# ChenJiahao031008/EAO-Fusion

Hardware: AMD Instinct MI355X
Metric: ORB kpts/s (640x480, 1k feat) + local-BA residuals/s (20 KF x 3k pts) (higher is better)
Workload: dtype u8; 1 GPU; ORBextractor FAST+rBRIEF, 640x480, 8-level pyramid, nFeatures 1000, batch=64 synthetic frames per GPU (BASELINE configs[1]); parallelism=frames sharded per GPU, no data-path collective

## Files before the change

eao_fusion_amd/csrc/orb.hip:

```cpp
#include "orb_internal.h"

using namespace eao::orb;

namespace {

__constant__ __align__(16) signed char c_pattern[1024] = {
#include "orb_pattern.inc"
};

constexpr int kResizeRows = 4;
__device__ __forceinline__ unsigned udot2w(unsigned a, unsigned b) {
    typedef unsigned short us2 __attribute__((ext_vector_type(2)));
    return __builtin_amdgcn_udot2(__builtin_bit_cast(us2, a), __builtin_bit_cast(us2, b), 0u, false);
}

struct ResizeLevel { int w, h, pitch, off; };
struct ResizeArgs {
    ResizeLevel D, S;
    double invX, invY;
    int srcIsInput;
    int pyrFrameBytes;
    int G;
    float invG;
    int frameAffinity;
// ... 535 lines not shown
    if (MODE == 1) {
        const unsigned a = e.left ? L[0] : L[1], b = e.left ? L[1] : L[2];
        W0 = __builtin_amdgcn_perm(L[1], L[0], e.selA);
        W1 = __builtin_amdgcn_perm(b, a, e.selB);
        W2 = __builtin_amdgcn_perm(b, a, e.selC);
    }
    constexpr unsigned T0 = 18u | 34u << 8 | 49u << 16 | 55u << 24, T1 = 49u | 34u << 8 | 18u << 16;
    hres[0] = __builtin_amdgcn_udot4(__builtin_amdgcn_alignbyte(W1, W0, 1), T0, __builtin_amdgcn_udot4(__builtin_amdgcn_alignbyte(W2, W1, 1), T1, 0, false), false);
    hres[1] = __builtin_amdgcn_udot4(__builtin_amdgcn_alignbyte(W1, W0, 2), T0, __builtin_amdgcn_udot4(__builtin_amdgcn_alignbyte(W2, W1, 2), T1, 0, false), false);
    hres[2] = __builtin_amdgcn_udot4(__builtin_amdgcn_alignbyte(W1, W0, 3), T0, __builtin_amdgcn_udot4(__builtin_amdgcn_alignbyte(W2, W1, 3), T1, 0, false), false);
    hres[3] = __builtin_amdgcn_udot4(W1, T0, __builtin_amdgcn_udot4(W2, T1, 0, false), false);
}

template <int MODE>
__device__ __forceinline__ void blur_strip(const uint8_t* __restrict__ src, int pitch, uint8_t* __restrict__ dst, int dpitch, int x4, int y0, int w, int h) {
    BlurEdge e = {};
    if (MODE == 1) e = blur_edge(x4, w);
    constexpr int NP = (kBlurRows + 6) / 2;
    constexpr int PF = MODE == 2 ? 1 : 3;
    unsigned raw[NP][2][3];
    auto fetch = [&](int m) {
#pragma unroll
        for (int q = 0; q < 2; q++) {
            int t = y0 - 3 + 2 * m + q;
            t = t < 0 ? -t : t;
            t = min(t, 2 * h - 2 - t);
            blur_load<MODE>(src, __umul24(t, pitch), x4, w, e, raw[m][q]);
        }
    };
#pragma unroll
    for (int m = 0; m < PF; m++) fetch(m);
    unsigned P[4][4];
#pragma unroll
    for (int m = 0; m < NP; m++) {
        if (m + PF < NP) fetch(m + PF);
        unsigned hr[2][4];
        blur_hpass<MODE>(raw[m][0], e, hr[0]);
        blur_hpass<MODE>(raw[m][1], e, hr[1]);
#pragma unroll
        for (int i = 0; i < 4; i++) P[m & 3][i] = hr[0][i] | (hr[1][i] << 16);
        if (m >= 3) {
#pragma unroll
            for (int q = 0; q < 2; q++) {
                const unsigned K0 = q ? 18u << 16 : (18u | 34u << 16), K1 = q ? (34u | 49u << 16) : (49u | 55u << 16),
                               K2 = q ? (55u | 49u << 16) : (49u | 34u << 16), K3 = q ? (34u | 18u << 16) : 18u;
                unsigned sv[4];
#pragma unroll
                for (int i = 0; i < 4; i++)
                    sv[i] = udot2(P[(m - 3) & 3][i], K0, udot2(P[(m - 2) & 3][i], K1, udot2(P[(m - 1) & 3][i], K2, udot2(P[m & 3][i], K3, 32768u))));
                const u16x2 lim = {255, 255};
                const u16x2 pa = __builtin_elementwise_min(__builtin_bit_cast(u16x2, __builtin_amdgcn_perm(sv[1], sv[0], 0x07060302u)), lim);
                const u16x2 pb = __builtin_elementwise_min(__builtin_bit_cast(u16x2, __builtin_amdgcn_perm(sv[3], sv[2], 0x07060302u)), lim);
                const unsigned packed = __builtin_amdgcn_perm(__builtin_bit_cast(unsigned, pb), __builtin_bit_cast(unsigned, pa), 0x06040200u);
                const int y = y0 + 2 * (m - 3) + q;
                *reinterpret_cast<unsigned*>(dst + (unsigned)(__umul24(y, dpitch) + x4)) = packed;
            }
        }
    }
}

__global__ __launch_bounds__(256) void k_blur7(const Geom* __restrict__ g, ImgSrc s, uint8_t* __restrict__ blur, int f0, int src0Aligned, int frameAffinity) {
    const int lane = threadIdx.x & 31;
    int f = blockIdx.y, bxi = blockIdx.x;
    if (frameAffinity) {
        const unsigned b = blockIdx.x + gridDim.x * blockIdx.y, xcd = b & 7, slot = b >> 3;
        f = (int)(xcd + 8 * (slot / gridDim.x)); bxi = (int)(slot % gridDim.x);
    }
    f += f0;
    int l = 0;
    while (l + 1 < g->nlevels && bxi >= g->L[l + 1].tileBase) l++;
    const LevelGeom L = g->L[l];
    const int strip = (bxi - L.tileBase) * kBlurStripsPerWg + (int)(threadIdx.x >> 5);
    const int x4 = (strip % L.tilesX) * kBlurSegW + lane * 4;
    const int y0 = (strip / L.tilesX) * kBlurRows;
    if (x4 >= L.w || y0 >= L.h) return;
    int pitch;
    const uint8_t* src = level_ptr(g, s, l, f, &pitch);
    uint8_t* dst = blur + (long long)f * g->pyrFrameBytes + L.off;
    if (l == 0 && !src0Aligned) blur_strip<2>(src, pitch, dst, L.pitch, x4, y0, L.w, L.h);
    else if (__any(x4 < 4 || x4 + 7 > L.w)) blur_strip<1>(src, pitch, dst, L.pitch, x4, y0, L.w, L.h);
    else blur_strip<0>(src, pitch, dst, L.pitch, x4, y0, L.w, L.h);
}

__device__ __forceinline__ int half_sum_i32(int v, int half) {
    v += __builtin_amdgcn_update_dpp(0, v, 0xB1, 0xF, 0xF, true);
    v += __builtin_amdgcn_update_dpp(0, v, 0x4E, 0xF, 0xF, true);
    v += __builtin_amdgcn_update_dpp(0, v, 0x141, 0xF, 0xF, true);
    v += __builtin_amdgcn_update_dpp(0, v, 0x140, 0xF, 0xF, true);
    v += __builtin_amdgcn_update_dpp(0, v, 0x142, 0xA, 0xF, true);
    const int lo = __builtin_amdgcn_readlane(v, 31), hi = __builtin_amdgcn_readlane(v, 63);
    return half ? hi : lo;
}

constexpr int kUmaxTab[16] = {15, 15, 15, 15, 14, 14, 14, 13, 13, 12, 11, 10, 9, 8, 6, 3};

__device__ __forceinline__ void sincos_f32_via_f64(float angle, float* sn, float* cs) {
    const double x = (double)angle;
    const int k = (int)(x * 0.63661977236758134308 + 0.5);
    const double kd = (double)k;
    const double r = (x - kd * 1.57079632673412561417e+00) - kd * 6.07710050650619224932e-11;
    const double z = r * r;
    const double ps = -1.66666666666666324348e-01 + z * (8.33333333332248946124e-03 + z * (-1.98412698298579493134e-04 +
                      z * (2.75573137070700676789e-06 + z * (-2.50507602534068634195e-08 + z * 1.58969099521155010221e-10))));
    const double sr = r + r * z * ps;
    const double pc = 4.16666666666666019037e-02 + z * (-1.38888888888741095749e-03 + z * (2.48015872894767294178e-05 +
                      z * (-2.75573143513906633035e-07 + z * (2.08757232129817482790e-09 + z * -1.13596475577881948265e-11))));
    const double cr = 1.0 - 0.5 * z + z * z * pc;
    double sv = (k & 1) ? cr : sr, cv = (k & 1) ? sr : cr;
    if (k & 2) sv = -sv;
    if ((k + 1) & 2) cv = -cv;
    *sn = (float)sv;
    *cs = (float)cv;
}

__device__ __forceinline__ float fast_atan2_deg(float y, float x) {
    const float p1 = 0.9997878412794807f * (float)(180 / 3.1415926535897932384626433832795);
    const float p3 = -0.3258083974640975f * (float)(180 / 3.1415926535897932384626433832795);
    const float p5 = 0.1555786518463281f * (float)(180 / 3.1415926535897932384626433832795);
    const float p7 = -0.04432655554792128f * (float)(180 / 3.1415926535897932384626433832795);
    const float eps = (float)2.2204460492503131e-16;
    const float ax = fabsf(x), ay = fabsf(y);
    const bool ge = ax >= ay;
    const float c = (ge ? ay : ax) / ((ge ? ax : ay) + eps);
    const float c2 = c * c;
    const float poly = (((p7 * c2 + p5) * c2 + p3) * c2 + p1) * c;
    float a = ge ? poly : 90.f - poly;
    if (x < 0) a = 180.f - a;
    if (y < 0) a = 360.f - a;
    return a;
}

constexpr int kDescKp = 8;
constexpr int kPR = 18, kPW = 10, kPRows = 2 * kPR + 1, kPLoads = (kPRows + 2) / 3;
constexpr int kMR = 15, kMW = 9, kMRows = 2 * kMR + 1, kMLoads = (kMRows + 2) / 3;

__global__ __launch_bounds__(256) void k_orient_describe(const Geom* __restrict__ g, ImgSrc s, const uint8_t* __restrict__ blur,
                                                         const unsigned* __restrict__ levelkps, const int* __restrict__ levelcnt,
                                                         eao_keypoint* __restrict__ kps, uint8_t* __restrict__ desc,
                                                         int* __restrict__ nout, int cap, int f0, int nlevels, int lFirst, int lEnd, int writeN,
                                                         int frameAffinity) {
    const int lane = threadIdx.x & 63, wv = __builtin_amdgcn_readfirstlane(threadIdx.x >> 6);
    const int hl = lane & 31, half = lane >> 5;
    const int bx = frameAffinity ? (int)(blockIdx.x >> 3) : (int)blockIdx.x;
    const int fy = frameAffinity ? (int)((blockIdx.x & 7) + 8 * blockIdx.y) : (int)blockIdx.y;
    int p = bx * 4 + wv;
    const int f = fy + f0;
    int total, l, kbase, pbase, cntl;
    {
        int cinc = lane < lEnd ? levelcnt[f * nlevels + lane] : 0;
        int pinc = (cinc + 1) >> 1;
        cinc += __builtin_amdgcn_update_dpp(0, cinc, 0x111, 0xF, 0xF, true);
        pinc += __builtin_amdgcn_update_dpp(0, pinc, 0x111, 0xF, 0xF, true);
        cinc += __builtin_amdgcn_update_dpp(0, cinc, 0x112, 0xF, 0xF, true);
        pinc += __builtin_amdgcn_update_dpp(0, pinc, 0x112, 0xF, 0xF, true);
        cinc += __builtin_amdgcn_update_dpp(0, cinc, 0x114, 0xF, 0xF, true);
        pinc += __builtin_amdgcn_update_dpp(0, pinc, 0x114, 0xF, 0xF, true);
        cinc += __builtin_amdgcn_update_dpp(0, cinc, 0x118, 0xF, 0xF, true);
        pinc += __builtin_amdgcn_update_dpp(0, pinc, 0x118, 0xF, 0xF, true);
        total = __builtin_amdgcn_readlane(cinc, 15);
        if (lFirst > 0) p += __builtin_amdgcn_readlane(pinc, lFirst - 1);
        l = (int)__popcll(__ballot(lane < nlevels && pinc <= p));
        const int lprev = min(l, kMaxLevels) - 1;
        pbase = l > 0 ? __builtin_amdgcn_readlane(pinc, lprev) : 0;
        kbase = l > 0 ? __builtin_amdgcn_readlane(cinc, lprev) : 0;
        cntl = __builtin_amdgcn_readlane(cinc, min(l, kMaxLevels - 1)) - kbase;
    }
// ... 148 lines not shown
    const int row = (int)vL;
    const float minZ = A.mb, minD = -3, maxD = A.mbf / minZ;
    const float minU = uL - maxD, maxU = uL - minD;
    float outU = -1.0f, outD = -1.0f;
    int outS = -1;
    if (!(maxU < 0)) {
        const uint4 a0 = A.dl[2 * iL], a1 = A.dl[2 * iL + 1];
        unsigned best = 0xFFFFFFFFu;
        for (int iR = lane; iR < A.nr; iR += 64) {
            const eao_keypoint kr = A.kr[iR];
            const float r = 2.0f * A.scale[kr.octave];
            const int maxr = (int)ceilf(kr.y + r), minr = (int)floorf(kr.y - r);
            if (row < minr || row > maxr) continue;
            if (kr.octave < levelL - 1 || kr.octave > levelL + 1) continue;
            if (!(kr.x >= minU && kr.x <= maxU)) continue;
            const uint4 b0 = A.dr[2 * iR], b1 = A.dr[2 * iR + 1];
            const unsigned d = __popc(a0.x ^ b0.x) + __popc(a0.y ^ b0.y) + __popc(a0.z ^ b0.z) + __popc(a0.w ^ b0.w) +
                               __popc(a1.x ^ b1.x) + __popc(a1.y ^ b1.y) + __popc(a1.z ^ b1.z) + __popc(a1.w ^ b1.w);
            best = min(best, (d << 16) | (unsigned)iR);
        }
        for (int dlt = 32; dlt >= 1; dlt >>= 1) best = min(best, (unsigned)__shfl_xor((int)best, dlt));
        const int bestDist = (int)(best >> 16);
        if (best != 0xFFFFFFFFu && bestDist < refc::TH_HIGH) {
            const int bestIdxR = (int)(best & 0xFFFF);
            const float uR0 = A.kr[bestIdxR].x;
            const float sf = A.invScale[levelL];
            const int suL = (int)roundf(uL * sf), svL = (int)roundf(vL * sf), suR0 = (int)roundf(uR0 * sf);
            const int w = 5, Lw = 5;
            int pl, pr;
            const uint8_t* imgL = level_ptr(g, sl, levelL, A.frame, &pl);
            const uint8_t* imgR = level_ptr(g, sr, levelL, A.frame, &pr);
            const int lw = g->L[levelL].w, lh = g->L[levelL].h;
            const float iniu = (float)(suR0 + Lw - w), endu = (float)(suR0 + Lw + w + 1);
            if (!(iniu < 0 || endu >= (float)lw)) {
                const int cL = px_reflect(imgL, pl, lw, lh, suL, svL);
                int dL0 = 0, dL1 = 0, px0x = 0, px0y = 0, px1x = 0, px1y = 0;
                const bool has1 = lane + 64 < 121;
                px0y = lane / 11; px0x = lane - px0y * 11;
                dL0 = px_reflect(imgL, pl, lw, lh, suL - w + px0x, svL - w + px0y) - cL;
                if (has1) {
                    px1y = (lane + 64) / 11; px1x = lane + 64 - px1y * 11;
                    dL1 = px_reflect(imgL, pl, lw, lh, suL - w + px1x, svL - w + px1y) - cL;
                }
                int dists[11];
                int bestSad = 0x7FFFFFFF, bestinc = 0;
#pragma unroll
                for (int inc = -5; inc <= 5; inc++) {
                    const int cR = px_reflect(imgR, pr, lw, lh, suR0 + inc, svL);
                    int sacc = abs(dL0 - (px_reflect(imgR, pr, lw, lh, suR0 + inc - w + px0x, svL - w + px0y) - cR));
                    if (has1) sacc += abs(dL1 - (px_reflect(imgR, pr, lw, lh, suR0 + inc - w + px1x, svL - w + px1y) - cR));
                    for (int dlt = 32; dlt >= 1; dlt >>= 1) sacc += __shfl_xor(sacc, dlt);
                    dists[inc + 5] = sacc;
                    if (sacc < bestSad) { bestSad = sacc; bestinc = inc; }
                }
                if (!(bestinc == -Lw || bestinc == Lw)) {
                    float dist1 = 0, dist2 = 0, dist3 = 0;
#pragma unroll
                    for (int k = 0; k < 11; k++) {
                        if (k == Lw + bestinc - 1) dist1 = (float)dists[k];
                        if (k == Lw + bestinc) dist2 = (float)dists[k];
                        if (k == Lw + bestinc + 1) dist3 = (float)dists[k];
                    }
                    const float deltaR = (dist1 - dist3) / (2.0f * (dist1 + dist3 - 2.0f * dist2));
                    if (!(deltaR < -1 || deltaR > 1)) {
                        float bestuR = A.scale[levelL] * ((float)suR0 + (float)bestinc + deltaR);
                        float disparity = uL - bestuR;
                        if (disparity >= 0 && disparity < maxD) {
                            if (disparity <= 0) { disparity = 0.01f; bestuR = uL - 0.01f; }
                            outD = A.mbf / disparity;
                            outU = bestuR;
                            outS = bestSad;
                        }
                    }
                }
            }
        }
    }
    if (lane == 0) { A.uRight[iL] = outU; A.depth[iL] = outD; A.sad[iL] = outS; }
}

namespace eao {
namespace orb {

eao_status enqueue(eao_orb* h, const uint8_t* d_img, int pitch0, long long fs0, int batch, eao_keypoint* d_kps,
                   uint8_t* d_desc, int cap, int* d_n, hipStream_t st) {
    const Geom& g = h->geom;
    eao::Range rAll("eao_orb_extract: enqueue");
    ImgSrc s;
    s.img0 = d_img; s.pitch0 = pitch0; s.fs0 = fs0; s.pyr = h->d_pyr.p;
    h->lastSrc = s; h->lastBatch = batch; h->lastComplete = false; h->pyrFrame = -1;
    const bool prof = h->profiling;
    hipEvent_t* ev = nullptr;
    if (prof) {
        if (h->evUsed + kProfEvents > h->evs.size()) {
            const size_t old = h->evs.size();
            h->evs.resize(old + kProfEvents * 16, nullptr);
            for (size_t i = old; i < h->evs.size(); i++) EAO_HIP(hipEventCreate(&h->evs[i]));
        }
        ev = &h->evs[h->evUsed];
        h->evUsed += kProfEvents;
        EAO_HIP(hipEventRecord(ev[0], st));
    }
    eao_status so;
    if (h->evLastValid && h->lastStream != st) {
        if ((so = order_behind_last_call(h, st))) return so;
    }
    h->lastStream = st;
    EAO_HIP(hipEventRecord(h->evStart, st));
    const hipStream_t ss = h->side;
    const int cells0 = g.L[0].nCells;
    const bool early0 = !prof && g.nlevels > 1 && g.L[0].cellBase == 0 && cells0 < g.totalCells;
    const int aff = (batch & 7) == 0 ? 1 : 0;
    auto fast = [&](hipStream_t str, int first, int end) {
        eao::Range rg("orb: FAST cells");
        const bool whole = first == 0 && end == g.totalCells, narrow = g.fastStride == 48;
        auto* kern = whole ? (narrow ? k_fast_cells<true, 48> : k_fast_cells<true, kTileStrideWide>)
                           : (narrow ? k_fast_cells<false, 48> : k_fast_cells<false, kTileStrideWide>);
        hipLaunchKernelGGL(kern, dim3(128 * ((end - first + 127) / 128), batch), dim3(64), g.fastLdsBytes, str, h->d_geom.p, h->d_cells.p, s,
                           h->d_cellcand.p, h->d_cellcnt.p, 0, first, end, aff);
    };
    const int mid = early0 && batch >= 48 && g.nlevels > 3 ? 3 : 0;
    const bool qtEarly = mid > 0 && batch <= 96;
    const int src0Aligned = ((((uintptr_t)s.img0 | (uintptr_t)s.pitch0 | (uintptr_t)(batch > 1 ? s.fs0 : 0)) & 3) == 0) ? 1 : 0;
    auto quadtree = [&](hipStream_t str, int lFirst, int nLev) {
        eao::Range rg("orb: quad-tree");
        launch_quadtree(h, str, batch, 0, lFirst, nLev);
    };
    auto blur = [&]() -> eao_status {
        EAO_HIP(hipStreamWaitEvent(ss, h->evFork, 0));
        if (prof) EAO_HIP(hipEventRecord(ev[6], ss));
        { eao::Range rg("orb: blur"); hipLaunchKernelGGL(k_blur7, dim3(g.totalTiles, batch), dim3(256), 0, ss, h->d_geom.p, s, h->d_blur.p, 0, src0Aligned, aff); }
        if (prof) EAO_HIP(hipEventRecord(ev[7], ss));
        EAO_HIP(hipEventRecord(h->evJoin, ss));
        return EAO_OK;
    };
    auto describe = [&](hipStream_t str, int lFirst, int lEnd, int writeN) {
        eao::Range rg("orb: orientation + description");
        int pairs = 0;
        for (int l = lFirst; l < lEnd; l++) pairs += eao::cdiv(g.L[l].listCap, 2);
        const int gx = std::max(1, eao::cdiv(std::min(pairs, eao::cdiv(cap, 2) + g.nlevels), 4));
        hipLaunchKernelGGL(k_orient_describe, aff ? dim3(8 * gx, batch / 8) : dim3(gx, batch), dim3(256), 0, str,
                           h->d_geom.p, s, h->d_blur.p, h->d_levelkps.p, h->d_levelcnt.p, d_kps, d_desc, d_n, cap, 0, g.nlevels, lFirst, lEnd, writeN, aff);
    };
    if (h->pyrFused && batch <= 32) {
        auto pyramid = [&] {
            eao::Range rg("orb: pyramid");
            hipLaunchKernelGGL(k_pyramid_fused, dim3(h->pyr.tilesX * h->pyr.tilesY, 1, batch), dim3(kPyrThreads), h->pyrLds, st, h->pyr, s, 0);
        };
        if (prof) {
            pyramid();
            EAO_HIP(hipEventRecord(ev[1], st));
            EAO_HIP(hipEventRecord(h->evFork, st));
            if ((so = blur())) return so;
            EAO_HIP(hipStreamWaitEvent(st, h->evJoin, 0));
            EAO_HIP(hipEventRecord(ev[9], st));
            fast(st, 0, g.totalCells);
            EAO_HIP(hipEventRecord(ev[2], st));
            quadtree(st, 0, g.nlevels);
            EAO_HIP(hipEventRecord(ev[3], st));
            EAO_HIP(hipEventRecord(ev[4], st));
        } else {
            EAO_HIP(hipStreamWaitEvent(ss, h->evStart, 0));
            fast(ss, 0, cells0);
            quadtree(ss, 0, 1);
            pyramid();
            EAO_HIP(hipEventRecord(h->evFork, st));
            if ((so = blur())) return so;
            fast(st, cells0, g.totalCells);
            quadtree(st, 1, g.nlevels - 1);
            EAO_HIP(hipStreamWaitEvent(st, h->evJoin, 0));
        }
    } else {
        if (early0) {
            EAO_HIP(hipStreamWaitEvent(ss, h->evStart, 0));
            fast(ss, 0, cells0);
        }
        for (int l = 1; l < g.nlevels; l++) {
            const int G4 = eao::cdiv(g.L[l].w, 4);
            ResizeArgs ra;
            ra.G = G4; ra.invG = 1.0f / (float)G4;
            ra.D = {g.L[l].w, g.L[l].h, g.L[l].pitch, g.L[l].off};
            ra.S = {g.L[l - 1].w, g.L[l - 1].h, g.L[l - 1].pitch, g.L[l - 1].off};
            ra.invX = 1. / ((double)g.L[l].w / g.L[l - 1].w); ra.invY = 1. / ((double)g.L[l].h / g.L[l - 1].h);
            ra.srcIsInput = l == 1; ra.pyrFrameBytes = g.pyrFrameBytes;
            ra.frameAffinity = aff;
            { eao::Range rg("orb: pyramid"); hipLaunchKernelGGL(k_resize, dim3(eao::cdiv(G4 * eao::cdiv(g.L[l].h, kResizeRows), 64), 1, batch), dim3(64), 0, st, ra, s, 0); }
            if (l == mid - 1) {
                EAO_HIP(hipEventRecord(h->evMid, st));
                EAO_HIP(hipStreamWaitEvent(ss, h->evMid, 0));
                fast(ss, cells0, g.L[mid].cellBase);
                if (qtEarly) quadtree(ss, 0, mid);
            }
        }
        if (early0 && !qtEarly) EAO_HIP(hipEventRecord(h->evFast0, ss));
        if (prof) {
            EAO_HIP(hipEventRecord(ev[1], st));
            EAO_HIP(hipEventRecord(h->evFork, st));
            if ((so = blur())) return so;
            EAO_HIP(hipStreamWaitEvent(st, h->evJoin, 0));
            EAO_HIP(hipEventRecord(ev[9], st));
            fast(st, 0, g.totalCells);
            EAO_HIP(hipEventRecord(ev[2], st));
        } else {
            EAO_HIP(hipEventRecord(h->evFork, st));
            fast(st, early0 ? (mid ? g.L[mid].cellBase : cells0) : 0, g.totalCells);
            if ((so = blur())) return so;
            if (early0 && !qtEarly) EAO_HIP(hipStreamWaitEvent(st, h->evFast0, 0));
        }
        quadtree(st, qtEarly ? mid : 0, g.nlevels - (qtEarly ? mid : 0));
        if (prof) EAO_HIP(hipEventRecord(ev[3], st));
        EAO_HIP(hipStreamWaitEvent(st, h->evJoin, 0));
        if (prof) EAO_HIP(hipEventRecord(ev[4], st));
    }
    describe(st, 0, g.nlevels, 1);
// ... 200 lines not shown
```

eao_fusion_amd/csrc/orb_host.hip:

```cpp
#include "orb_internal.h"

using namespace eao::orb;

namespace eao {
namespace orb {

eao_status build_geometry(eao_orb* h, int W, int H) {
    const eao_orb_cfg& c = h->cfg;
    Geom& g = h->geom;
    std::memset(&g, 0, sizeof(g));
    g.nlevels = c.nlevels; g.W = W; g.H = H;
    g.iniTh = c.ini_th_fast; g.minTh = c.min_th_fast;
    for (int i = 0; i < 16; i++) g.umax[i] = h->umax[i];
    h->cells.clear();
    int off = 0, kpBase = 0, candBase = 0, tileBase = 0, maxCell = 0, scanCap = 0, maxList = 0, maxSw = 0, maxSh = 0;
    for (int l = 0; l < c.nlevels; l++) {
        LevelGeom& L = g.L[l];
        const float s = h->invScale[l];
        L.w = cv_round((float)W * s);
        L.h = cv_round((float)H * s);
        EAO_REQUIRE(L.w < 4096 && L.h < 4096, "level %d is %dx%d: coordinates are packed in 12 bits", l, L.w, L.h);
        const int maxBX = L.w - kEdge + 3, maxBY = L.h - kEdge + 3;
        const float width = (float)(maxBX - kMinBorder), height = (float)(maxBY - kMinBorder);
        const int nCols = (int)(width / (float)refc::FAST_CELL), nRows = (int)(height / (float)refc::FAST_CELL);
// ... 84 lines not shown
                    capv[c.nlevels - 1] = std::max(capv[c.nlevels - 1], r1 - r0);
                    for (int l = 1; l < c.nlevels; l++) { table[(size_t)l * nT + col].x = o0[l]; table[(size_t)l * nT + col].y = o1[l]; }
                    table[(size_t)(c.nlevels - 1) * nT + col].z = r0; table[(size_t)(c.nlevels - 1) * nT + col].w = r1;
                    for (int l = c.nlevels - 1; l >= 1; l--) {
                        int q0 = l > 1 ? o0[l - 1] : 0x7FFFFFFF, q1 = l > 1 ? o1[l - 1] : 0;
                        if (r1 > r0) {
                            const double inv = isX ? P.L[l].invX : P.L[l].invY;
                            const int sn = isX ? g.L[l - 1].w : g.L[l - 1].h;
                            q0 = std::min(q0, pyr_src_ofs(r0, inv, sn));
                            q1 = std::max(q1, std::min(pyr_src_ofs(r1 - 1, inv, sn) + 1, sn - 1) + 1);
                        }
                        if (q0 > q1) q0 = q1 = 0;
                        capv[l - 1] = std::max(capv[l - 1], q1 - q0);
                        table[(size_t)(l - 1) * nT + col].z = q0; table[(size_t)(l - 1) * nT + col].w = q1;
                        r0 = q0; r1 = q1;
                    }
                }
            };
            axis(P.tilesX, kPyrTW, true, capW);
            axis(P.tilesY, kPyrTH, false, capH);
            size_t lds = 0;
            int coefCap = 1;
            for (int l = 0; l < c.nlevels; l++) {
                P.L[l].ldsW = ((capW[l] + 3) & ~3) + 16; P.L[l].ldsH = capH[l] + 1;
                P.L[l].ldsOff = (int)lds;
                lds += ((size_t)P.L[l].ldsW * P.L[l].ldsH + 15) & ~(size_t)15;
                coefCap = std::max(coefCap, std::max(capW[l], capH[l]));
            }
            coefCap = (coefCap + 7) & ~3;
            P.coefOff = (int)lds; P.coefCap = coefCap;
            lds += (size_t)coefCap * 16;
            h->pyrLds = lds;
            h->pyrFused = lds <= 64 * 1024 && h->cfg.scale_factor <= 2.0f;
            for (int l = 1; l < c.nlevels; l++)
                if (P.L[l].invX > 2.0 || P.L[l].invY > 2.0) h->pyrFused = false;
            if (h->pyrFused) {
                std::vector<int2> cxv, cyv;
                for (int l = 1; l < c.nlevels; l++) {
                    P.L[l].coefXOff = (int)cxv.size(); P.L[l].coefYOff = (int)cyv.size();
                    for (int d = 0; d < g.L[l].w; d++) { int o; unsigned w2; resize_coef_host(d, P.L[l].invX, g.L[l - 1].w, true, &o, &w2); cxv.push_back(make_int2(o, (int)w2)); }
                    for (int d = 0; d < g.L[l].h; d++) { int o; unsigned w2; resize_coef_host(d, P.L[l].invY, g.L[l - 1].h, false, &o, &w2); cyv.push_back(make_int2(o, (int)w2)); }
                }
                eao_status st2 = h->d_pyrRanges.reserve(table.size());
                if (st2) return st2;
                if ((st2 = h->d_pyrCoef.reserve(cxv.size() + cyv.size()))) return st2;
                EAO_HIP(hipMemcpy(h->d_pyrRanges.p, table.data(), table.size() * sizeof(int4), hipMemcpyHostToDevice));
                EAO_HIP(hipMemcpy(h->d_pyrCoef.p, cxv.data(), cxv.size() * sizeof(int2), hipMemcpyHostToDevice));
                EAO_HIP(hipMemcpy(h->d_pyrCoef.p + cxv.size(), cyv.data(), cyv.size() * sizeof(int2), hipMemcpyHostToDevice));
                P.ranges = h->d_pyrRanges.p;
                P.coefX = h->d_pyrCoef.p; P.coefY = h->d_pyrCoef.p + cxv.size();
            }
        }
    }
    g.scanCap = scanCap;
    g.fastMaxTested = std::max(1, (maxSw - 6) * (maxSh - 6));
    g.fastStride = maxSw + 3 <= 48 ? 48 : kTileStrideWide;
    g.fastTileBytes = ((maxSh * g.fastStride) + 15) & ~15;
    g.fastLdsBytes = g.fastTileBytes + ((2 * g.fastMaxTested + 15) & ~15) + ((((maxSw - 4) * (maxSh - 4)) + 15) & ~15) + 64;
    h->quadLds = (size_t)maxList * (2 * sizeof(short4) + sizeof(int) * kQtNodeInts) + (size_t)scanCap * sizeof(int);
    g.qtNodesGlobal = 0; g.qtNodeFrameBytes = 0;
    if (h->quadLds > 100 * 1024) {
        g.qtNodesGlobal = 1;
        long long noff = 0;
        for (int l = 0; l < c.nlevels; l++) {
            g.L[l].nodeOff = noff;
            noff += (long long)align256((size_t)g.L[l].listCap * (2 * sizeof(short4) + sizeof(int) * kQtNodeInts) + (size_t)scanCap * sizeof(int));
        }
        g.qtNodeFrameBytes = noff;
        h->quadLds = 0;
    }
    h->quadLds = (h->quadLds + 15) & ~(size_t)15;
    g.qtKeysOff = (int)h->quadLds;
    const size_t kQtLdsCand = std::min<size_t>(8192, std::max<size_t>(2048, ((size_t)h->cfg.nfeatures * 4 + 63) & ~(size_t)63));
    g.qtLdsCand = (int)std::min<size_t>(kQtLdsCand, h->quadLds < 76 * 1024 ? (76 * 1024 - h->quadLds) / 6 : 0) & ~7;
    h->quadLds += (size_t)g.qtLdsCand * 6;
    if (g.qtNodesGlobal) { g.qtLdsCand = 0; h->quadLds = 0; }
    {
        float cf[7]; double sum = 0;
        for (int i = 0; i < 7; i++) { double x = i - 3; cf[i] = (float)std::exp(-0.5 / 4.0 * x * x); sum += cf[i]; }
        const int expect[7] = {18, 34, 49, 55, 49, 34, 18};
        for (int i = 0; i < 7; i++)
            if (cv_round((double)(float)(cf[i] * (1. / sum)) * 256.0) != expect[i]) { eao::set_error("gaussian taps mismatch"); return EAO_ERR_INTERNAL; }
    }
    { eao_status st = h->d_geom.reserve(1); if (st) return st; }
    EAO_HIP(hipMemcpyAsync(h->d_geom.p, &g, sizeof(Geom), hipMemcpyHostToDevice, h->stream));
    { eao_status st = h->d_cells.reserve(h->cells.size()); if (st) return st; }
    EAO_HIP(hipMemcpyAsync(h->d_cells.p, h->cells.data(), h->cells.size() * sizeof(CellDesc), hipMemcpyHostToDevice, h->stream));
    EAO_HIP(eao::wait_latency(h->stream));
    { eao_status sq = quadtree_reserve_lds(h->quadLds); if (sq) return sq; }
    h->geomValid = true;
    h->batchCap = 0;
    return EAO_OK;
}

eao_status ensure(eao_orb* h, int W, int H, int batch, hipStream_t caller) {
    eao_status st = eao::require_device();
    if (st) return st;
    if (!h->stream && batch > 0) {
        int least = 0, greatest = 0, p = 0;
        const bool follow = (uintptr_t)caller != kNoCallerStream && !(getenv("EAO_STREAM_PRIORITY") && !atoi(getenv("EAO_STREAM_PRIORITY"))) &&
                            hipDeviceGetStreamPriorityRange(&least, &greatest) == hipSuccess && least != greatest && hipStreamGetPriority(caller, &p) == hipSuccess;
        (void)hipGetLastError();
        auto make = [&](hipStream_t* q) -> hipError_t {
            if ((uintptr_t)caller == kNoCallerStream) return eao::create_stream(q, eao::StreamClass::Latency);
            if (!follow || p == 0) return hipStreamCreateWithFlags(q, hipStreamNonBlocking);
            return hipStreamCreateWithPriority(q, hipStreamNonBlocking, p);
        };
        EAO_HIP(make(&h->stream));
        EAO_HIP(hipEventCreateWithFlags(&h->evStart, hipEventDisableTiming));
        EAO_HIP(hipEventCreateWithFlags(&h->evLast, hipEventDisableTiming));
        EAO_HIP(make(&h->spacer));
        EAO_HIP(make(&h->side));
        for (hipEvent_t* e : {&h->evFork, &h->evFast0, &h->evMid, &h->evJoin}) EAO_HIP(hipEventCreateWithFlags(e, hipEventDisableTiming));
    }
    if (!h->d_dbg && getenv("EAO_DEBUG_STAMPS")) {
        EAO_HIP(hipMalloc(&h->d_dbg, 16 * kMaxLevels * sizeof(long long)));
        EAO_HIP(hipMemset(h->d_dbg, 0, 16 * kMaxLevels * sizeof(long long)));
    }
    if (!h->geomValid || h->geom.W != W || h->geom.H != H) {
        st = build_geometry(h, W, H);
        if (st) return st;
    }
    if (batch > h->batchCap) {
        const Geom& g = h->geom;
        const size_t B = batch;
#define RES(buf, cnt) do { st = h->buf.reserve(cnt); if (st) return st; } while (0)
        RES(d_pyr, B * g.pyrFrameBytes);
        RES(d_blur, B * g.pyrFrameBytes);
        RES(d_cellcand, B * (size_t)g.totalCells * g.cellCap);
        RES(d_cellcnt, B * g.totalCells);
        RES(d_cand, B * (size_t)g.totalCandCap);
        RES(d_nodeof, B * (size_t)g.totalCandCap);
        if (g.qtNodesGlobal) RES(d_qtnodes, B * (size_t)g.qtNodeFrameBytes);
        RES(d_levelkps, B * (size_t)g.totalKpCap);
        RES(d_levelcnt, B * g.nlevels);
        RES(d_candcnt, B * g.nlevels);
#undef RES
        h->batchCap = batch;
    }
    return EAO_OK;
}

eao_status order_behind_last_call(eao_orb* h, hipStream_t st) {
    if (h->evLastRecorded) EAO_HIP(hipStreamWaitEvent(st, h->evLast, 0));
    else EAO_HIP(hipDeviceSynchronize());
    h->everyCallEvent = true;
    return EAO_OK;
}

void stream_release(eao_orb* h) {
    for (eao_orb::StreamSlot& sl : h->slots) {
        if (sl.evOut && sl.submitted) (void)hipEventSynchronize(sl.evOut);
        if (sl.pinIn) (void)hipHostFree(sl.pinIn);
        if (sl.pinOut) (void)hipHostFree(sl.pinOut);
        if (sl.dIn) (void)hipFree(sl.dIn);
        if (sl.dOut) (void)hipFree(sl.dOut);
        if (sl.evIn) (void)hipEventDestroy(sl.evIn);
        if (sl.evOut) (void)hipEventDestroy(sl.evOut);
        if (sl.evDone) (void)hipEventDestroy(sl.evDone);
    }
    h->slots.clear();
    for (hipStream_t* q : {&h->sUp, &h->sRun, &h->sDown})
        if (*q) { (void)hipStreamSynchronize(*q); (void)hipStreamDestroy(*q); *q = nullptr; }
}

eao_status wait_last_extraction(eao_orb* h) {
// ... 365 lines not shown
```

eao_fusion_amd/csrc/orb_internal.h:

```cpp
#pragma once

#include <algorithm>
#include <atomic>
#include <cmath>
#include <cstdlib>
#include <cstring>
#include <vector>

#include "common.h"


namespace eao {
namespace orb {

constexpr int kMaxLevels = 16;
constexpr int kEdge = refc::EDGE_THRESHOLD;
constexpr int kMinBorder = kEdge - 3;
constexpr int kTile = 72;
constexpr int kTileStrideWide = 80;
constexpr int kMaxIni = 16;
constexpr size_t kPinnedOutMax = 1 << 20;
constexpr int kFastXcdRun = 0;

struct LevelGeom {
    int w, h, pitch, off;
    int cellBase, nCells;
    int quota;
    int nIni, boxH;
    float hX;
    int listCap;
    int kpBase;
    int candBase, candCap;
    int tileBase, tilesX;
    long long nodeOff;
    int scaledPatch;
    float scale;
};

struct Geom {
    int nlevels, W, H;
    int totalCells, cellCap;
    int totalKpCap, totalCandCap, totalTiles;
    int pyrFrameBytes;
    int iniTh, minTh;
    int scanCap;
    int qtLdsCand, qtKeysOff;
    int qtNodesGlobal;
    long long qtNodeFrameBytes;
    int fastMaxTested, fastTileBytes, fastLdsBytes, fastStride;
    int umax[16];
    LevelGeom L[kMaxLevels];
};

struct CellDesc {
    short level, x0, y0, sw, sh, offX, offY, pad;
};

struct ImgSrc {
    const uint8_t* img0;
    int pitch0;
    long long fs0;
    uint8_t* pyr;
};

__device__ __forceinline__ const uint8_t* level_ptr(const Geom* g, const ImgSrc& s, int l, int f, int* pitch) {
    if (l == 0) {
        *pitch = s.pitch0;
        return s.img0 + (long long)f * s.fs0;
    }
    *pitch = g->L[l].pitch;
    return s.pyr + (long long)f * g->pyrFrameBytes + g->L[l].off;
}

constexpr int kPyrTW = 128, kPyrTH = 32;
constexpr int kPyrThreads = 256;
struct PyrLevel { int w, h, pitch, off; double invX, invY; int ldsOff, ldsW, ldsH; int coefXOff, coefYOff; };
struct PyrArgs {
    int nlevels, tilesX, tilesY, pyrFrameBytes;
    int coefOff;
    int coefCap;
    PyrLevel L[kMaxLevels];
    const int4* ranges;
    const int2* coefX;
    const int2* coefY;
};

constexpr int kQTSmall = 1024, kQTLarge = 256;
constexpr int kQtNodeInts = 2 + 2 + 2 + 4 + 4 + 5;

constexpr size_t kProfEvents = 10;


inline void resize_coef_host(int d, double inv, int slimit, bool clampHi, int* ofs, unsigned* wpair) {
    float fr = (float)(((double)d + 0.5) * inv - 0.5);
    int o = (int)std::floor(fr);
    fr -= (float)o;
    if (clampHi) {
        if (o < 0) { fr = 0; o = 0; }
        if (o >= slimit - 1) { fr = 0; o = slimit - 1; }
    }
    const int w0 = std::min(std::max((int)std::lrintf((1.f - fr) * 2048.f), -32768), 32767);
    const int w1 = std::min(std::max((int)std::lrintf(fr * 2048.f), -32768), 32767);
    *ofs = o;
    *wpair = ((unsigned)w0 & 0xFFFFu) | ((unsigned)w1 << 16);
}

__host__ __device__ inline int pyr_src_ofs(int d, double inv, int sn) {
    float fr = (float)(((double)d + 0.5) * inv - 0.5);
    int o = (int)floorf(fr);
    return o < 0 ? 0 : (o > sn - 1 ? sn - 1 : o);
}
__host__ __device__ inline int pyr_first_at_least(int bound, double inv, int sn, int dn) {
    if (bound <= 0) return 0;
    int d = (int)((double)bound / inv);
    d = d < 0 ? 0 : (d > dn ? dn : d);
    while (d > 0 && pyr_src_ofs(d - 1, inv, sn) >= bound) d--;
    while (d < dn && pyr_src_ofs(d, inv, sn) < bound) d++;
    return d;
}

constexpr int kBlurRows = 16;
constexpr int kBlurSegW = 128;
constexpr int kBlurStripsPerWg = 8;
inline int cv_round(double v) { return (int)std::lrint(v); }

}
}

struct eao_orb {
    using Geom = eao::orb::Geom; using CellDesc = eao::orb::CellDesc; using PyrArgs = eao::orb::PyrArgs; using ImgSrc = eao::orb::ImgSrc;
    eao_orb_cfg cfg;
    std::vector<float> scale, invScale, sigma2, invSigma2;
    std::vector<int> quota;
    int umax[16];
    Geom geom;
    bool geomValid = false;
    int batchCap = 0;
    std::vector<CellDesc> cells;
    size_t quadLds = 0;
    eao::DevBuf<int4> d_pyrRanges;
    eao::DevBuf<int2> d_pyrCoef;
    PyrArgs pyr;
    size_t pyrLds = 0;
    bool pyrFused = false;
    hipStream_t stream = nullptr;
    hipStream_t side = nullptr;
    hipStream_t spacer = nullptr;
    bool evLastValid = false;
    hipStream_t lastStream = nullptr;
    hipEvent_t evLast = nullptr;
    bool everyCallEvent = false, evLastRecorded = false;
    hipEvent_t evStart = nullptr, evFork = nullptr, evJoin = nullptr, evFast0 = nullptr, evMid = nullptr;
    eao::DevBuf<Geom> d_geom;
    eao::DevBuf<CellDesc> d_cells;
    eao::DevBuf<uint8_t> d_pyr, d_blur, d_in;
    eao::DevBuf<unsigned> d_cellcand, d_cand, d_levelkps;
    eao::DevBuf<unsigned short> d_nodeof;
    eao::DevBuf<unsigned char> d_qtnodes;
    eao::DevBuf<int> d_cellcnt, d_levelcnt, d_candcnt, d_nout;
    eao::DevBuf<eao_keypoint> d_kps;
    unsigned char* pinOut = nullptr;
    size_t pinOutCap = 0;
    unsigned char* pinUp = nullptr;
    size_t pinUpCap = 0;
    eao::DevBuf<uint8_t> d_desc;
    eao::DevBuf<float> d_xyr;
    eao::DevBuf<unsigned char> d_stereo;
    unsigned char* pinPyr = nullptr;
    size_t pinPyrCap = 0;
    eao_orb_level_view pyrViews[eao::orb::kMaxLevels] = {};
    int pyrFrame = -1, pyrBorder = -1;
    int autoPyrBorder = -1;
    bool lastComplete = false;
    ImgSrc lastSrc{};
    int lastBatch = 0;
    bool profiling = false;
    long long* d_dbg = nullptr;
    std::vector<hipEvent_t> evs;
    size_t evUsed = 0;
    struct StreamSlot {
        unsigned char* pinIn = nullptr; unsigned char* pinOut = nullptr;
        unsigned char* pinOutDev = nullptr;
        unsigned char* dIn = nullptr; unsigned char* dOut = nullptr;
        hipEvent_t evIn = nullptr, evDone = nullptr, evOut = nullptr;
        int batch = 0;
        bool submitted = false;
    };
    std::vector<StreamSlot> slots;
    hipStream_t sUp = nullptr, sRun = nullptr, sDown = nullptr;
    int sW = 0, sH = 0, sB = 0, sCap = 0, sPitch = 0;
    size_t sInBytes = 0, sOutBytes = 0, sOffK = 0, sOffD = 0;
};

namespace eao {
namespace orb {
constexpr uintptr_t kNoCallerStream = ~(uintptr_t)0;
eao_status ensure(eao_orb* h, int W, int H, int batch, hipStream_t caller = (hipStream_t)kNoCallerStream);
eao_status order_behind_last_call(eao_orb* h, hipStream_t st);
void stream_release(eao_orb* h);
eao_status wait_last_extraction(eao_orb* h);
eao_status upload_frames(eao_orb* h, const uint8_t* img, int width, int height, int stride, long long frame_stride, int batch);
eao_status enqueue(eao_orb* h, const uint8_t* d_img, int pitch0, long long fs0, int batch, eao_keypoint* d_kps, uint8_t* d_desc, int cap, int* d_n, hipStream_t st);
eao_status enqueue_pyramid_export(eao_orb* h, int frame, int border);
void launch_quadtree(const eao_orb* h, hipStream_t str, int nb, int f0, int lFirst, int nLev);
eao_status quadtree_reserve_lds(size_t bytes);
}
}
```

Before: 271.1 million kpts/s.

## Compute 7-tap Gaussian blur as int8 MFMA matrix products with precomputed tap tables

Adds a blur kernel that expresses the separable 7-tap Gaussian as two int8 MFMA matrix multiplies (horizontal then vertical) over 32x32 tiles. It uses host-built, deduplicated tap matrices that fold reflect-101 borders into the weights, and splits intermediates into hi/lo byte planes to keep exact integer results. The aim is to move blur arithmetic off the vector ALUs onto matrix cores. In exchange it adds LDS staging, table loads, and a VALU fallback for levels too small for the tiling. It is enabled by default and can be disabled with an environment variable.

```diff
diff --git a/eao_fusion_amd/csrc/orb.hip b/eao_fusion_amd/csrc/orb.hip
--- a/eao_fusion_amd/csrc/orb.hip
+++ b/eao_fusion_amd/csrc/orb.hip
@@ -641,6 +641,141 @@
     else blur_strip<0>(src, pitch, dst, L.pitch, x4, y0, L.w, L.h);
 }
 
+typedef int bm_v4i __attribute__((ext_vector_type(4)));
+typedef int bm_v16i __attribute__((ext_vector_type(16)));
+typedef bm_v4i bm_v4i_a4 __attribute__((aligned(4)));
+struct BlurMPacked { bm_v4i hi, lo; };
+
+constexpr int kBlurMLdsPitch = 80;
+__device__ __forceinline__ void blur_m_load(const uint8_t* __restrict__ src, int pitch, int h, int blk, unsigned ws, int lane, bm_v4i raw[2]) {
+#pragma unroll
+    for (int k = 0; k < 2; k++) {
+        const int y = min(max(kBlurMTile * blk + 16 * k + (lane >> 2), 0), h - 1);
+        raw[k] = *reinterpret_cast<const bm_v4i_a4*>(src + (unsigned)(__umul24(y, pitch) + ws + 16 * (lane & 3)));
+    }
+}
+
+__device__ __forceinline__ BlurMPacked blur_m_stage1(const bm_v4i raw[2], uint8_t* stage, int lane, bm_v4i tx0, bm_v4i tx1) {
+    const bm_v4i bias = {(int)0x80808080u, (int)0x80808080u, (int)0x80808080u, (int)0x80808080u};
+    bm_v16i z;
+#pragma unroll
+    for (int q = 0; q < 16; q++) z[q] = 0;
+    eao::wave_sync();
+#pragma unroll
+    for (int k = 0; k < 2; k++) *reinterpret_cast<bm_v4i*>(stage + (16 * k + (lane >> 2)) * kBlurMLdsPitch + 16 * (lane & 3)) = raw[k] ^ bias;
+    eao::wave_sync();
+    const uint8_t* fr = stage + (lane & 31) * kBlurMLdsPitch + 16 * (lane >> 5);
+    const bm_v4i a0 = *reinterpret_cast<const bm_v4i*>(fr), a1 = *reinterpret_cast<const bm_v4i*>(fr + 32);
+    bm_v16i X = __builtin_amdgcn_mfma_i32_32x32x32_i8(a0, tx0, z, 0, 0, 0);
+    X = __builtin_amdgcn_mfma_i32_32x32x32_i8(a1, tx1, X, 0, 0, 0);
+    BlurMPacked P;
+    const u16x2 k128 = {128, 128};
+#pragma unroll
+    for (int q = 0; q < 4; q++) {
+        const unsigned t = __builtin_amdgcn_perm((unsigned)X[4 * q + 1], (unsigned)X[4 * q], 0x05040100u);
+        const unsigned w = __builtin_amdgcn_perm((unsigned)X[4 * q + 3], (unsigned)X[4 * q + 2], 0x05040100u);
+        P.lo[q] = (int)__builtin_amdgcn_perm(w, t, 0x06040200u);
+        const unsigned t2 = __builtin_bit_cast(unsigned, __builtin_bit_cast(u16x2, t) + k128), w2 = __builtin_bit_cast(unsigned, __builtin_bit_cast(u16x2, w) + k128);
+        P.hi[q] = (int)__builtin_amdgcn_perm(w2, t2, 0x07050301u);
+    }
+    return P;
+}
+
+__device__ __forceinline__ void blur_m_stage2(const BlurMPacked& Pm, const BlurMPacked& Pc, const BlurMPacked& Pn, const bm_v4i ty[3], int lane,
+                                              uint8_t* __restrict__ dst, int dpitch, int x0, int b, int h, const bm_v16i& c) {
+    bm_v16i z;
+#pragma unroll
+    for (int q = 0; q < 16; q++) z[q] = 0;
+    bm_v16i ah = __builtin_amdgcn_mfma_i32_32x32x32_i8(Pm.hi, ty[0], z, 0, 0, 0);
+    bm_v16i al = __builtin_amdgcn_mfma_i32_32x32x32_i8(Pm.lo, ty[0], c, 0, 0, 0);
+    ah = __builtin_amdgcn_mfma_i32_32x32x32_i8(Pc.hi, ty[1], ah, 0, 0, 0);
+    al = __builtin_amdgcn_mfma_i32_32x32x32_i8(Pc.lo, ty[1], al, 0, 0, 0);
+    ah = __builtin_amdgcn_mfma_i32_32x32x32_i8(Pn.hi, ty[2], ah, 0, 0, 0);
+    al = __builtin_amdgcn_mfma_i32_32x32x32_i8(Pn.lo, ty[2], al, 0, 0, 0);
+    unsigned o[4];
+#pragma unroll
+    for (int q = 0; q < 4; q++) {
+        unsigned sv[4];
+#pragma unroll
+        for (int e = 0; e < 4; e++) sv[e] = ((unsigned)ah[4 * q + e] << 8) + (unsigned)al[4 * q + e];
+        const u16x2 lim = {255, 255};
+        const u16x2 pa = __builtin_elementwise_min(__builtin_bit_cast(u16x2, __builtin_amdgcn_perm(sv[1], sv[0], 0x07060302u)), lim);
+        const u16x2 pb = __builtin_elementwise_min(__builtin_bit_cast(u16x2, __builtin_amdgcn_perm(sv[3], sv[2], 0x07060302u)), lim);
+        o[q] = __builtin_amdgcn_perm(__builtin_bit_cast(unsigned, pb), __builtin_bit_cast(unsigned, pa), 0x06040200u);
+    }
+    const auto s02 = __builtin_amdgcn_permlane32_swap(o[0], o[2], false, false);
+    const auto s13 = __builtin_amdgcn_permlane32_swap(o[1], o[3], false, false);
+    const int y = kBlurMTile * b + (lane & 31);
+    if (y < h) *reinterpret_cast<uint4*>(dst + (unsigned)(__umul24(y, dpitch) + x0 + 16 * (lane >> 5))) = make_uint4(s02[0], s02[1], s13[0], s13[1]);
+}
+
+__global__ __launch_bounds__(256, 4) void k_blur7_mfma(const Geom* __restrict__ g, ImgSrc s, uint8_t* __restrict__ blur, const uint8_t* __restrict__ tab, int f0,
+                                                    int src0Aligned, int frameAffinity) {
+    int f = blockIdx.y, bxi = blockIdx.x;
+    if (frameAffinity) {
+        const unsigned b = blockIdx.x + gridDim.x * blockIdx.y, xcd = b & 7, slot = b >> 3;
+        f = (int)(xcd + 8 * (slot / gridDim.x)); bxi = (int)(slot % gridDim.x);
+    }
+    f += f0;
+    int l = 0;
+    while (l + 1 < g->nlevels && bxi >= g->L[l + 1].mTileBase) l++;
+    const LevelGeom L = g->L[l];
+    int pitch;
+    const uint8_t* src = level_ptr(g, s, l, f, &pitch);
+    uint8_t* dst = blur + (long long)f * g->pyrFrameBytes + L.off;
+    if (!L.mOk || (l == 0 && !src0Aligned)) {
+        const int lane = threadIdx.x & 31;
+        const int strip = (bxi - L.mTileBase) * kBlurStripsPerWg + (int)(threadIdx.x >> 5);
+        const int x4 = (strip % L.tilesX) * kBlurSegW + lane * 4;
+        const int y0 = (strip / L.tilesX) * kBlurRows;
+        if (x4 >= L.w || y0 >= L.h) return;
+        if (l == 0 && !src0Aligned) blur_strip<2>(src, pitch, dst, L.pitch, x4, y0, L.w, L.h);
+        else if (__any(x4 < 4 || x4 + 7 > L.w)) blur_strip<1>(src, pitch, dst, L.pitch, x4, y0, L.w, L.h);
+        else blur_strip<0>(src, pitch, dst, L.pitch, x4, y0, L.w, L.h);
+        return;
+    }
+    const int lane = threadIdx.x & 63;
+    const int task = __builtin_amdgcn_readfirstlane((bxi - L.mTileBase) * 4 + (int)(threadIdx.x >> 6));
+    int walkLen;
+    blur_m_walks(L.mBlocksY, &walkLen);
+    const int cx = task % L.mTilesX, b0 = (task / L.mTilesX) * walkLen;
+    if (b0 >= L.mBlocksY) return;
+    const int b1 = min(b0 + walkLen, L.mBlocksY);
+    const int2* idx = reinterpret_cast<const int2*>(tab);
+    const uint8_t* frag = tab + g->mFragOff;
+    const int2 xi = idx[L.mXIdx + cx];
+    const bm_v4i tx0 = *reinterpret_cast<const bm_v4i*>(frag + xi.y + lane * 16), tx1 = *reinterpret_cast<const bm_v4i*>(frag + xi.y + kBlurMFrag + lane * 16);
+    const unsigned ws = (unsigned)xi.x;
+    __shared__ __attribute__((aligned(16))) uint8_t sStage[4][kBlurMTile * kBlurMLdsPitch];
+    uint8_t* stage = sStage[threadIdx.x >> 6];
+    bm_v16i c2;
+#pragma unroll
+    for (int q = 0; q < 16; q++) c2[q] = 257 * (32768 + 128) + 32768;
+    asm volatile("" : "+v"(c2));
+    bm_v4i raw[2], ty[3];
+    int tyOff = -1;
+    BlurMPacked P[3];
+    P[0].hi = P[0].lo = bm_v4i{0, 0, 0, 0};
+    if (b0 > 0) { blur_m_load(src, pitch, L.h, b0 - 1, ws, lane, raw); P[0] = blur_m_stage1(raw, stage, lane, tx0, tx1); }
+    blur_m_load(src, pitch, L.h, b0, ws, lane, raw);
+    P[1] = blur_m_stage1(raw, stage, lane, tx0, tx1);
+    blur_m_load(src, pitch, L.h, b0 + 1, ws, lane, raw);
+#pragma unroll
+    for (int i = 0; i < kBlurMSeg; i++) {
+        const int b = b0 + i;
+        if (b >= b1) break;
+        P[(i + 2) % 3] = blur_m_stage1(raw, stage, lane, tx0, tx1);
+        if (b + 1 < b1) blur_m_load(src, pitch, L.h, b + 2, ws, lane, raw);
+        const int yo = idx[L.mYIdx + b].y;
+        if (yo != tyOff) {
+            tyOff = yo;
+#pragma unroll
+            for (int k = 0; k < 3; k++) ty[k] = *reinterpret_cast<const bm_v4i*>(frag + yo + k * kBlurMFrag + lane * 16);
+        }
+        blur_m_stage2(P[i % 3], P[(i + 1) % 3], P[(i + 2) % 3], ty, lane, dst, L.pitch, kBlurMTile * cx, b, L.h, c2);
+    }
+}
+
 __device__ __forceinline__ int half_sum_i32(int v, int half) {
     v += __builtin_amdgcn_update_dpp(0, v, 0xB1, 0xF, 0xF, true);
     v += __builtin_amdgcn_update_dpp(0, v, 0x4E, 0xF, 0xF, true);
@@ -955,6 +1090,8 @@
 namespace eao {
 namespace orb {
 
+static int blur_mfma_mode() { static const int mode = [] { const char* e = getenv("EAO_ORB_BLUR_MFMA"); return e ? atoi(e) : 1; }(); return mode; }
+
 eao_status enqueue(eao_orb* h, const uint8_t* d_img, int pitch0, long long fs0, int batch, eao_keypoint* d_kps,
                    uint8_t* d_desc, int cap, int* d_n, hipStream_t st) {
     const Geom& g = h->geom;
@@ -1002,7 +1139,12 @@
     auto blur = [&]() -> eao_status {
         EAO_HIP(hipStreamWaitEvent(ss, h->evFork, 0));
         if (prof) EAO_HIP(hipEventRecord(ev[6], ss));
-        { eao::Range rg("orb: blur"); hipLaunchKernelGGL(k_blur7, dim3(g.totalTiles, batch), dim3(256), 0, ss, h->d_geom.p, s, h->d_blur.p, 0, src0Aligned, aff); }
+        {
+            eao::Range rg("orb: blur");
+            if (g.mTotalTiles && blur_mfma_mode())
+                hipLaunchKernelGGL(k_blur7_mfma, dim3(g.mTotalTiles, batch), dim3(256), 0, ss, h->d_geom.p, s, h->d_blur.p, h->d_blurTab.p, 0, src0Aligned, aff);
+            else hipLaunchKernelGGL(k_blur7, dim3(g.totalTiles, batch), dim3(256), 0, ss, h->d_geom.p, s, h->d_blur.p, 0, src0Aligned, aff);
+        }
         if (prof) EAO_HIP(hipEventRecord(ev[7], ss));
         EAO_HIP(hipEventRecord(h->evJoin, ss));
         return EAO_OK;
diff --git a/eao_fusion_amd/csrc/orb_blur_tables.h b/eao_fusion_amd/csrc/orb_blur_tables.h
--- /dev/null
+++ b/eao_fusion_amd/csrc/orb_blur_tables.h
@@ -0,0 +1,122 @@
+#pragma once
+
+#include <cstdint>
+#include <cstring>
+#include <map>
+#include <string>
+#include <vector>
+
+namespace eao {
+namespace orb {
+
+constexpr int kBlurMTile = 32;
+constexpr int kBlurMWin = 64;
+constexpr int kBlurMSeg = 8;
+constexpr int kBlurMFrag = 1024;
+constexpr int kBlurTaps[7] = {18, 34, 49, 55, 49, 34, 18};
+
+struct BlurMLevelIn { int w, h, readable; };
+struct BlurMLevel {
+    int ok;
+    int tilesX, blocksY;
+    int xIdx, yIdx;
+};
+struct BlurMTables {
+    std::vector<BlurMLevel> level;
+    std::vector<int> idx;
+    std::vector<uint8_t> frag;
+    int maxEntry = 0;
+};
+
+inline int blur_reflect101(int p, int len) {
+    while (p < 0 || p >= len) p = p < 0 ? -p : 2 * len - 2 - p;
+    return p;
+}
+inline int blur_m_window_start(int cx, int readable) {
+    int ws = kBlurMTile * cx - 16;
+    if (ws > readable - kBlurMWin) ws = readable - kBlurMWin;
+    return ws < 0 ? 0 : ws;
+}
+#if defined(__HIPCC__)
+__host__ __device__
+#endif
+inline int blur_m_walks(int blocksY, int* len) {
+    const int n = (blocksY + kBlurMSeg - 1) / kBlurMSeg;
+    *len = (blocksY + n - 1) / n;
+    return n;
+}
+inline int blur_m_ty_slot(int rowInBlock, int* half) {
+    *half = (rowInBlock >> 2) & 1;
+    return (rowInBlock & 3) + 4 * (rowInBlock >> 3);
+}
+
+inline bool blur_m_tx(int cx, int w, int ws, uint8_t* out ) {
+    std::memset(out, 0, 2 * kBlurMFrag);
+    for (int c = 0; c < kBlurMTile; c++) {
+        const int x = kBlurMTile * cx + c;
+        if (x >= w) continue;
+        for (int t = 0; t < 7; t++) {
+            const int k = blur_reflect101(x - 3 + t, w) - ws;
+            if (k < 0 || k >= kBlurMWin) return false;
+            out[(k >> 5) * kBlurMFrag + (c + 32 * ((k >> 4) & 1)) * 16 + (k & 15)] += (uint8_t)kBlurTaps[t];
+        }
+    }
+    return true;
+}
+inline bool blur_m_ty(int b, int h, uint8_t* out ) {
+    std::memset(out, 0, 3 * kBlurMFrag);
+    for (int r = 0; r < kBlurMTile; r++) {
+        const int y = kBlurMTile * b + r;
+        if (y >= h) continue;
+        for (int t = 0; t < 7; t++) {
+            const int sy = blur_reflect101(y - 3 + t, h);
+            const int s = (sy >> 5) - (b - 1);
+            if (s < 0 || s > 2) return false;
+            int half;
+            const int j = blur_m_ty_slot(sy & 31, &half);
+            out[s * kBlurMFrag + (r + 32 * half) * 16 + j] += (uint8_t)kBlurTaps[t];
+        }
+    }
+    return true;
+}
+
+inline BlurMTables blur_m_build(const std::vector<BlurMLevelIn>& in) {
+    BlurMTables T;
+    std::map<std::string, int> seen;
+    auto intern = [&](const uint8_t* p, int bytes) {
+        for (int i = 0; i < bytes; i++) T.maxEntry = T.maxEntry > p[i] ? T.maxEntry : p[i];
+        const std::string key((const char*)p, (size_t)bytes);
+        auto it = seen.find(key);
+        if (it != seen.end()) return it->second;
+        const int off = (int)T.frag.size();
+        T.frag.insert(T.frag.end(), p, p + bytes);
+        seen.emplace(key, off);
+        return off;
+    };
+    std::vector<uint8_t> buf(3 * kBlurMFrag);
+    for (const BlurMLevelIn& L : in) {
+        BlurMLevel M{};
+        M.tilesX = (L.w + kBlurMTile - 1) / kBlurMTile;
+        M.blocksY = (L.h + kBlurMTile - 1) / kBlurMTile;
+        M.ok = L.w >= kBlurMWin && L.h >= kBlurMWin && L.readable >= L.w;
+        std::vector<int> idx;
+        for (int cx = 0; M.ok && cx < M.tilesX; cx++) {
+            const int ws = blur_m_window_start(cx, L.readable);
+            if (!blur_m_tx(cx, L.w, ws, buf.data())) { M.ok = 0; break; }
+            idx.push_back(ws); idx.push_back(intern(buf.data(), 2 * kBlurMFrag));
+        }
+        for (int b = 0; M.ok && b < M.blocksY; b++) {
+            if (!blur_m_ty(b, L.h, buf.data())) { M.ok = 0; break; }
+            idx.push_back(0); idx.push_back(intern(buf.data(), 3 * kBlurMFrag));
+        }
+        if (M.ok) {
+            M.xIdx = (int)T.idx.size() / 2; M.yIdx = M.xIdx + M.tilesX;
+            T.idx.insert(T.idx.end(), idx.begin(), idx.end());
+        }
+        T.level.push_back(M);
+    }
+    return T;
+}
+
+}
+}
diff --git a/eao_fusion_amd/csrc/orb_host.hip b/eao_fusion_amd/csrc/orb_host.hip
--- a/eao_fusion_amd/csrc/orb_host.hip
+++ b/eao_fusion_amd/csrc/orb_host.hip
@@ -190,6 +190,33 @@
         for (int i = 0; i < 7; i++)
             if (cv_round((double)(float)(cf[i] * (1. / sum)) * 256.0) != expect[i]) { eao::set_error("gaussian taps mismatch"); return EAO_ERR_INTERNAL; }
     }
+    {
+        std::vector<BlurMLevelIn> in;
+        for (int l = 0; l < c.nlevels; l++) in.push_back({g.L[l].w, g.L[l].h, l == 0 ? (g.L[l].w + 3) & ~3 : g.L[l].pitch});
+        const BlurMTables T = blur_m_build(in);
+        EAO_REQUIRE(T.maxEntry <= 127, "blur table entry %d does not fit int8", T.maxEntry);
+        int mBase = 0, any = 0;
+        for (int l = 0; l < c.nlevels; l++) {
+            LevelGeom& L = g.L[l];
+            const BlurMLevel& M = T.level[l];
+            L.mOk = M.ok; L.mTilesX = M.tilesX; L.mBlocksY = M.blocksY; L.mXIdx = M.xIdx; L.mYIdx = M.yIdx;
+            const int valu = eao::cdiv(L.tilesX * eao::cdiv(L.h, kBlurRows), kBlurStripsPerWg);
+            int walkLen;
+            const int mfma = eao::cdiv(M.tilesX * blur_m_walks(M.blocksY, &walkLen), 4);
+            L.mTileBase = mBase;
+            mBase += !M.ok ? valu : l == 0 ? std::max(valu, mfma) : mfma;
+            any |= M.ok;
+        }
+        g.mTotalTiles = any ? mBase : 0;
+        g.mFragOff = (int)((T.idx.size() * sizeof(int) + kBlurMFrag - 1) / kBlurMFrag * kBlurMFrag);
+        if (any) {
+            std::vector<uint8_t> blob((size_t)g.mFragOff + T.frag.size(), 0);
+            std::memcpy(blob.data(), T.idx.data(), T.idx.size() * sizeof(int));
+            std::memcpy(blob.data() + g.mFragOff, T.frag.data(), T.frag.size());
+            { eao_status st = h->d_blurTab.reserve(blob.size()); if (st) return st; }
+            EAO_HIP(hipMemcpy(h->d_blurTab.p, blob.data(), blob.size(), hipMemcpyHostToDevice));
+        }
+    }
     { eao_status st = h->d_geom.reserve(1); if (st) return st; }
     EAO_HIP(hipMemcpyAsync(h->d_geom.p, &g, sizeof(Geom), hipMemcpyHostToDevice, h->stream));
     { eao_status st = h->d_cells.reserve(h->cells.size()); if (st) return st; }
diff --git a/eao_fusion_amd/csrc/orb_internal.h b/eao_fusion_amd/csrc/orb_internal.h
--- a/eao_fusion_amd/csrc/orb_internal.h
+++ b/eao_fusion_amd/csrc/orb_internal.h
@@ -8,6 +8,7 @@
 #include <vector>
 
 #include "common.h"
+#include "orb_blur_tables.h"
 
 
 namespace eao {
@@ -32,6 +33,9 @@
     int kpBase;
     int candBase, candCap;
     int tileBase, tilesX;
+    int mOk, mTileBase;
+    int mTilesX, mBlocksY;
+    int mXIdx, mYIdx;
     long long nodeOff;
     int scaledPatch;
     float scale;
@@ -41,6 +45,7 @@
     int nlevels, W, H;
     int totalCells, cellCap;
     int totalKpCap, totalCandCap, totalTiles;
+    int mTotalTiles, mFragOff;
     int pyrFrameBytes;
     int iniTh, minTh;
     int scanCap;
@@ -154,6 +159,7 @@
     eao::DevBuf<Geom> d_geom;
     eao::DevBuf<CellDesc> d_cells;
     eao::DevBuf<uint8_t> d_pyr, d_blur, d_in;
+    eao::DevBuf<uint8_t> d_blurTab;
     eao::DevBuf<unsigned> d_cellcand, d_cand, d_levelkps;
     eao::DevBuf<unsigned short> d_nodeof;
     eao::DevBuf<unsigned char> d_qtnodes;
```

Measured after the change: 278.6 million kpts/s (median of 6 runs). 1.03x the previous value.
